# giuvecchio/PyPBR

Hardware: AMD Instinct MI355X
Metric: Mpixels/s Cook-Torrance eval, 4K maps (higher is better)
Workload: dtype f32

## Files before the change

### __graft_entry__.py

```python
import os
import subprocess
import sys

ROOT = os.path.dirname(os.path.abspath(__file__))
if ROOT not in sys.path:
    sys.path.insert(0, ROOT)


def build() -> None:
    subprocess.check_call(["make", "-s", "-j4", "-C", os.path.join(ROOT, "pypbr_amd", "csrc")])
    subprocess.check_call(["make", "-s", "-C", os.path.join(ROOT, "pypbr_amd", "csrc"), "torch_ops"])
    subprocess.check_call(["make", "-s", "-C", os.path.join(ROOT, "oracle")])
    boxcal_src, boxcal_so = os.path.join(ROOT, "tools", "boxcal.hip"), os.path.join(ROOT, "tools", "libboxcal.so")
    if not os.path.exists(boxcal_so) or os.path.getmtime(boxcal_so) < os.path.getmtime(boxcal_src):
        try:
            subprocess.check_call([os.environ.get("HIPCC", "/opt/rocm/bin/hipcc"), "-O3", "--offload-arch=gfx950", "-shared", "-fPIC", boxcal_src, "-o", boxcal_so])
        except (OSError, subprocess.CalledProcessError) as e:
            print("warning: tools/libboxcal.so (bench-side calibration helper, optional) did not build: %s" % e, file=sys.stderr)
    sys.path.insert(0, os.path.join(ROOT, "tools"))
    import check_isa
    report = check_isa.check()
    print("ISA check ok: %d hand-scheduled kernel instantiations; %s" % (sum(1 for r in report if "<" in r.split("vgpr")[0]), report[-1][:120]))
    import pypbr_amd
    from pypbr_amd import _native
    lib = _native.lib()
    for sym in _native.EXPORTS:
        getattr(lib, sym)
    assert lib.pbr_abi_version() == _native.ABI_VERSION
    from pypbr_amd import torch_ops
    assert torch_ops.available(), "pypbr_amd/_pbr_torch_ops.so did not build or load"
    import torch
    for op in ("cook_torrance", "cook_torrance_backward", "fold_gradient", "srgb_to_linear", "linear_to_srgb",
               "metallic_to_diffuse_specular", "diffuse_specular_to_basecolor_metallic", "colour_backward",
               "metallic_to_diffuse_specular_backward", "diffuse_specular_to_basecolor_metallic_backward", "resize", "resize_backward",
               "normal_from_height", "normal_from_height_backward", "normal_transform", "normal_transform_backward",
               "remap_planes", "remap_planes_backward"):
        getattr(torch.ops.pbr_hip, op)
    print("build ok: %s (ABI %d), pypbr_amd %s" % (_native.LIB_PATH, lib.pbr_abi_version(), pypbr_amd.__version__))


def smoke() -> None:
    import torch
    sys.path.insert(0, os.path.join(ROOT, "oracle"))
    import torch_oracle
    from pypbr_amd.materials import BasecolorMetallicMaterial
    from pypbr_amd.models import CookTorranceBRDF

    assert torch.cuda.is_available(), "smoke() needs a ROCm device"
    g = torch.Generator().manual_seed(2024)
    H, W = 96, 128
    albedo = torch.rand(3, H, W, generator=g)
    nxy = torch.rand(2, H, W, generator=g) - 0.5
    normal = torch.cat([nxy, torch.ones(1, H, W)], 0)
    normal = normal / normal.norm(dim=0, keepdim=True)
    rough = torch.rand(1, H, W, generator=g) * 0.85 + 0.15
    metal = torch.rand(1, H, W, generator=g)
    view, light, inten = torch.tensor([0.0, 0.0, 1.0]), torch.tensor([0.1, 0.1, 1.0]), torch.tensor([1.0, 1.0, 1.0])

    mat = BasecolorMetallicMaterial(albedo=albedo, normal=normal, roughness=rough, metallic=metal).to("cuda:0")
    out = CookTorranceBRDF(light_type="point")(mat, view, light, inten, 1.0)
    torch.cuda.synchronize()
    assert out.shape == (3, H, W) and out.device.type == "cuda"
    ref = torch_oracle.cook_torrance(albedo, normal, rough, metal, None, view=view, light=light, intensity=inten,
                                     light_type="point", light_size=1.0)
    err = (out.cpu() - ref).abs().max().item()
    print("smoke: max |hip - oracle| = %.3e over %d values" % (err, ref.numel()))
    assert err <= 1e-5, err


if __name__ == "__main__":
    build()
    if len(sys.argv) > 1 and sys.argv[1] == "smoke":
        smoke()
```

### pypbr_amd/_caches.py

```python
import os
import threading
import weakref
from typing import Optional

import torch

CACHING = {"device_maps": False, "parameters": False, "decode_verdicts": False}
for _tok, _key in (("maps", "device_maps"), ("params", "parameters"), ("decode", "decode_verdicts")):
    if _tok in os.environ.get("PBR_CACHE", "").split(","):
        CACHING[_key] = True


def set_caching(device_maps: Optional[bool] = None, parameters: Optional[bool] = None, decode_verdicts: Optional[bool] = None) -> dict:
    old = dict(CACHING)
    for key, v in (("device_maps", device_maps), ("parameters", parameters), ("decode_verdicts", decode_verdicts)):
        if v is not None:
            CACHING[key] = bool(v)
    return old


def version_of(t: torch.Tensor):
    try:
        return None if t.is_inference() else t._version
    except RuntimeError:
        return None


def weak_refs(tensors):
    return tuple(None if t is None else weakref.ref(t) for t in tensors)


def same_tensors(refs, tensors) -> bool:
    return len(refs) == len(tensors) and all((r is None and t is None) or (r is not None and r() is t) for r, t in zip(refs, tensors))


def host_values(v):
    if isinstance(v, torch.Tensor):
        return None if v.is_cuda or v.requires_grad else v.tolist()
    if isinstance(v, (list, tuple)):
        return [list(r) if isinstance(r, (list, tuple)) else r for r in v]
    return None


class VersionMemo:

    def __init__(self, limit: int = 64):
        self.limit, self._entries = limit, {}

    def get(self, t, version):
        e = self._entries.get(id(t))
        return e[2] if e is not None and e[0]() is t and e[1] == version else None

    def put(self, t, version, payload):
        for k in [k for k, e in self._entries.items() if e[0]() is None]:
            del self._entries[k]
        if len(self._entries) >= self.limit:
            self._entries.clear()
        self._entries[id(t)] = (weakref.ref(t), version, payload)

    def __len__(self):
        return len(self._entries)

    def clear(self):
        self._entries.clear()


class ValueMemo:

    def __init__(self, limit: int = 256):
        self.limit, self._entries = limit, {}

    def get(self, key, make):
        hit = self._entries.get(key)
        if hit is None:
            hit = make()
            if len(self._entries) >= self.limit:
                self._entries.clear()
            self._entries[key] = hit
        return hit

    def __len__(self):
        return len(self._entries)

    def clear(self):
        self._entries.clear()


class KeptPlan:
    __slots__ = ("plan", "maps", "values", "lock", "out_shape")

    def __init__(self, plan, maps, values, out_shape=None):
        self.plan, self.maps, self.values, self.out_shape = plan, weak_refs(maps), values, out_shape
        self.lock = threading.Lock()

    @classmethod
    def adopt(cls, plan, maps, values, out_shape=None):
        if plan._param_block is not None or not all(p is None or (t is not None and p.data_ptr() == t.data_ptr()) for p, t in zip(plan._keep, maps)):
            return None
        plan._keep = ()
        return cls(plan, maps, values, out_shape)

    def describes(self, maps) -> bool:
        return same_tensors(self.maps, maps)

    def try_acquire(self) -> bool:
        return self.lock.acquire(False)

    def release(self):
        self.lock.release()

    def refresh(self, values) -> bool:
        if values != self.values:
            if not self.plan.refill(*values):
                return False
            self.values = values
        return True
```

### pypbr_amd/models.py

```python
import collections
import os
import weakref
from abc import ABC
from typing import Optional

import torch
import torch.nn as nn
from torch import Tensor

from . import _native
from . import functional as F_
from ._caches import KeptPlan, host_values, same_tensors, weak_refs
from .materials import MaterialBase, _normalised


DEVICE_CACHE_CAP = int(os.environ.get("PBR_DEVICE_CACHE_CAP", str(4 << 30)))
_DEVICE_CACHES = collections.OrderedDict()


def _touch_device_cache(material):
    if id(material) in _DEVICE_CACHES:
        _DEVICE_CACHES.move_to_end(id(material))


def _register_device_cache(material, nbytes):
    _DEVICE_CACHES.pop(id(material), None)
    for key in [k for k, (ref, _) in _DEVICE_CACHES.items() if ref() is None or "_device_cache" not in ref().__dict__]:
        del _DEVICE_CACHES[key]
    _DEVICE_CACHES[id(material)] = (weakref.ref(material), nbytes)
    total = sum(n for _, n in _DEVICE_CACHES.values())
    while total > DEVICE_CACHE_CAP and len(_DEVICE_CACHES) > 1:
        _, (ref, n) = _DEVICE_CACHES.popitem(last=False)
        if ref() is not None:
            ref().__dict__.pop("_device_cache", None)
        total -= n


def _upload_together(tensors, compute):
    host = [i for i, t in enumerate(tensors) if t is not None and t.device.type == "cpu"]
    moved = [None if t is None else (t if t.device == compute or t.device.type == "cpu" else t.to(compute)) for t in tensors]
    if host:
        views, _ = F_.upload_packed([tensors[i] for i in host], compute)
        for i, v in zip(host, views):
            moved[i] = v
    return tuple(moved)


class BRDFModel(nn.Module, ABC):
    """Abstract base class for BRDF models (cooktorrance.py:27-30)."""


class CookTorranceBRDF(BRDFModel):

    def __init__(self, light_type: str = "point", override_device: torch.device = None):
        super().__init__()
        self.light_type = light_type.lower()
        if self.light_type not in ["directional", "point"]:
            raise ValueError(
                f"Unsupported light_type: {self.light_type}. Must be 'directional' or 'point'."
            )
        self.override_device = override_device

    @staticmethod
    def _staged(material, maps, blend, compute):
        tensors = tuple(maps) + tuple(blend or ())
        if any(t is not None and t.requires_grad for t in tensors):
            moved = tuple(None if t is None else t.to(compute) for t in tensors)
            return moved[:5], (None if blend is None else moved[5:])
        versions = tuple(None if t is None else F_.version_of(t) for t in tensors)
        wanted = (F_.CACHING["device_maps"] or material.__dict__.get("_cache_on_device", False))
        cacheable = wanted and all(v is not None for t, v in zip(tensors, versions) if t is not None)
        at, seen, refs, moved = (material.__dict__.get("_device_cache") if cacheable else None) or (None, None, (), None)
        if moved is not None and at == compute and seen == versions and same_tensors(refs, tensors):
            _touch_device_cache(material)
        else:
            moved = _upload_together(tensors, compute)
            if cacheable:
                material.__dict__["_device_cache"] = (compute, versions, weak_refs(tensors), moved)
                _register_device_cache(material, sum(t.numel() * t.element_size() for t in moved if t is not None))
        return moved[:5], (None if blend is None else moved[5:])

    PLAN_REUSE = True

    def _reuse_plan(self, material, view_dir, light, intensity, light_size, return_srgb):
        d = material.__dict__
        store = d.get("_store")
        if store is None or d.get("_lazy_blend") is not None or d.get("_raw_normal") or self.override_device is not None:
            return None
        vals = (host_values(view_dir), host_values(light), host_values(intensity))
        if vals[0] is None or vals[1] is None or vals[2] is None:
            return None
        albedo, normal, rough = store.get("albedo"), store.get("normal", False), store.get("roughness")
        metallic = store.get("metallic")
        specular = store.get("specular") if metallic is None else None
        if (albedo is None or normal is False or rough is None or (metallic is None and specular is None) or not albedo.is_cuda
                or albedo.device != material.device):
            return None
        maps = (albedo, normal, rough, metallic, specular)
        grad = torch.is_grad_enabled()
        for t in maps:
            if t is not None and (t.device != albedo.device or t.dtype.itemsize > 4 or not t.is_floating_point() or (grad and t.requires_grad)
                                  or t.stride(-1) != 1 or t.stride(-2) != t.shape[-1]):
                return None
        key = (self.light_type, light_size, bool(return_srgb), bool(material.albedo_is_srgb), bool(getattr(material, "specular_is_srgb", True)),
               d.get("_lazy_tile", (1, 1)),
               tuple((id(t), t.data_ptr(), t.shape, t.dtype, t.stride()) if t is not None else None for t in maps))
        kept_key, kept = d.get("_plan_cache") or (None, None)
        if kept is not None and (kept_key != key or not kept.describes(maps)):
            d.pop("_plan_cache", None)
            kept = None
        if kept is None:
            if d.get("_plan_seen") != key:
                d["_plan_seen"] = key
                return None
            return key
        if not kept.try_acquire():
            return None
        plan = kept.plan
        try:
            if not kept.refresh(vals):
                return key
            dev = plan.device
            out = torch.empty(kept.out_shape, dtype=torch.float32, device=dev)
            plan.out = out
            plan.desc.out = out.data_ptr()
            if torch.cuda.current_device() == dev.index:
                plan.launch()
            else:
                with torch.cuda.device(dev):
                    plan.launch()
            return out[0] if plan._squeeze else out
        finally:
            plan.out = None
            kept.release()

    def forward(self, material, view_dir: Tensor, light_dir_or_position: Tensor, light_intensity: Tensor,
                light_size: Optional[float] = None, return_srgb: bool = True) -> Tensor:
        reuse_key = None
        if self.PLAN_REUSE and isinstance(material, MaterialBase):
            got = self._reuse_plan(material, view_dir, light_dir_or_position, light_intensity, light_size, return_srgb)
            if isinstance(got, torch.Tensor):
                return got
            reuse_key = got
        out_device = _normalised(self.override_device or material.device)

        pending = material.__dict__.get("_lazy_blend")
        blend = None
        if pending is not None:
            first, (second, mask) = material.__dict__["_store"], pending
            albedo, normal, roughness = first["albedo"], first["normal"], first["roughness"]
            metallic, specular = first.get("metallic"), None
            if metallic is None:
                specular = first["specular"]
            specular_is_srgb = bool(getattr(material, "specular_is_srgb", True))
            blend = (second["albedo"], second["normal"], second["roughness"], second.get("metallic") if metallic is not None else None,
                     second.get("specular") if metallic is None else None, mask)
        else:
            store = material.__dict__.get("_store") if isinstance(material, MaterialBase) else None
            if store is not None and material._has_pending():
                store = {**store, **material._resident(keep=False)}

            def probe(name):
                if store is None:
                    return getattr(material, name)
                if name not in store:
                    raise AttributeError(f"'{type(material).__name__}' object has no attribute '{name}'")
                return store[name]

            def has(name):
                return (name in store) if store is not None else hasattr(material, name)

            roughness = probe("roughness")
            normal = probe("normal")
            metallic = specular = None
            specular_is_srgb = True
            if has("metallic") and probe("metallic") is not None:
                metallic = probe("metallic")
            elif has("specular") and probe("specular") is not None:
                specular = probe("specular")
                specular_is_srgb = bool(getattr(material, "specular_is_srgb", True))
            else:
                raise ValueError("Material must have either 'metallic' or 'specular' property.")
            albedo = store.get("albedo") if store is not None else material._maps.get("albedo")
            if albedo is None:
                raise AttributeError(f"'{type(material).__name__}' material has no albedo map")

        if out_device.type == "cuda":
            compute = out_device
        else:
            _native.require_device()
            compute = torch.device("cuda", torch.cuda.current_device())

        maps = (albedo, normal, roughness, metallic, specular)
        if any(t is not None and t.device != compute for t in maps + (blend or ())):
            maps, blend = self._staged(material, maps, blend, compute)
        kw = dict(view_dir=view_dir, light=light_dir_or_position, light_intensity=light_intensity, light_type=self.light_type,
                  light_size=light_size, albedo_is_srgb=bool(material.albedo_is_srgb), specular_is_srgb=specular_is_srgb,
                  return_srgb=return_srgb, tile=getattr(material, "lazy_tile", (1, 1)))
        if reuse_key is not None and blend is None and albedo.numel() > 0:
            plan = F_.plan_cook_torrance(*maps, **kw)
            with torch.cuda.device(plan.device):
                color = plan.launch()
            kept = KeptPlan.adopt(plan, maps, (host_values(view_dir), host_values(light_dir_or_position), host_values(light_intensity)),
                                  tuple(plan.out.shape))
            if kept is not None:
                material.__dict__["_plan_cache"] = (reuse_key, kept)
            plan.out = None
            return color
        color = F_.cook_torrance(*maps, blend=blend, **kw)
        if color.device == out_device:
            return color
        return F_.to_host(color, out_device) if out_device.type == "cpu" else color.to(out_device)
```

### pypbr_amd/torch_ops.py

```python
import os

import torch

_HERE = os.path.dirname(os.path.abspath(__file__))
LIB_PATH = os.path.join(_HERE, "_pbr_torch_ops.so")
_loaded = None


def available() -> bool:
    global _loaded
    if _loaded is None:
        _loaded = False
        if os.environ.get("PBR_NO_TORCH_OPS") != "1" and os.path.exists(LIB_PATH):
            from . import _native
            _native.lib()
            try:
                torch.ops.load_library(LIB_PATH)
                _register()
                _loaded = True
            except (OSError, RuntimeError) as e:
                import warnings
                warnings.warn("pypbr_amd: %s does not load against torch %s (%s); using the ctypes binding of libpbr_hip.so. "
                              "Rebuild with `make -C pypbr_amd/csrc torch_ops`." % (LIB_PATH, torch.__version__, str(e).splitlines()[0]),
                              RuntimeWarning, stacklevel=2)
    return _loaded


def _out_extent(albedo, tile_y, tile_x, y_offset, rows):
    B, _, H, W = albedo.shape
    if tile_y == 1 and tile_x == 1:
        return B, H, W
    return B, (rows if rows > 0 else tile_y * H - y_offset), tile_x * W


def _register():
    lib = torch.library

    @lib.register_fake("pbr_hip::cook_torrance")
    def _(albedo, normal, roughness, metallic, specular, view_dir, lights, intensities, light_size, light_type, albedo_is_srgb,
          specular_is_srgb, convert_to_diffuse_specular, return_srgb, y_offset=0, height_total=0, tile_y=1, tile_x=1, rows=0,
          half_result=False):
        B, H, W = _out_extent(albedo, tile_y, tile_x, y_offset, rows)
        return albedo.new_empty((B, 3, H, W), dtype=torch.float16 if half_result else torch.float32)

    @lib.register_fake("pbr_hip::cook_torrance_backward")
    def _(grad_out, albedo, normal, roughness, metallic, specular, view_dir, lights, intensities, light_size, light_type,
          albedo_is_srgb, specular_is_srgb, convert_to_diffuse_specular, return_srgb, y_offset, height_total, tile_y, tile_x, rows,
          want_albedo, want_normal, want_roughness, want_metallic, want_specular, want_params):
        B, H, W = _out_extent(albedo, tile_y, tile_x, y_offset, rows)
        maps = [t for t in (albedo, normal, roughness, metallic, specular) if t is not None]
        shared = B > 1 and any(t.shape[0] == 1 for t in maps)
        if (tile_y, tile_x) != (1, 1) and not want_params and not shared:
            H, W = albedo.shape[-2:]

        def buf(want, c):
            return albedo.new_empty((B, c, H, W)) if want else albedo.new_empty((0,))
        n_lights = lights.numel() // 3
        return (buf(want_albedo, 3), buf(want_normal and normal is not None, 3), buf(want_roughness, 1),
                buf(want_metallic and metallic is not None, 1), buf(want_specular and metallic is None, 3),
                albedo.new_empty((3 + 6 * n_lights,) if want_params else (0,), dtype=torch.float32))

    @lib.register_fake("pbr_hip::fold_gradient")
    def _(src, h, w, fold_batch):
        return src.new_empty((1 if fold_batch else src.shape[0], src.shape[1], h, w))

    for name in ("srgb_to_linear", "linear_to_srgb"):
        lib.register_fake("pbr_hip::" + name)(lambda texture: torch.empty_like(texture))
    lib.register_fake("pbr_hip::metallic_to_diffuse_specular")(
        lambda albedo, metallic, albedo_is_srgb: (torch.empty_like(albedo), torch.empty_like(albedo)))
    lib.register_fake("pbr_hip::diffuse_specular_to_basecolor_metallic")(
        lambda diffuse, specular, albedo_is_srgb: (torch.empty_like(diffuse), torch.empty_like(diffuse)))

    lib.register_fake("pbr_hip::colour_backward")(lambda texture, grad_out, to_linear: torch.empty_like(texture))
    lib.register_fake("pbr_hip::metallic_to_diffuse_specular_backward")(
        lambda albedo, metallic, g_diffuse, g_specular, albedo_is_srgb: (torch.empty_like(albedo), torch.empty_like(metallic)))
    lib.register_fake("pbr_hip::diffuse_specular_to_basecolor_metallic_backward")(
        lambda diffuse, specular, g_basecolor, g_metallic, albedo_is_srgb: (torch.empty_like(diffuse), torch.empty_like(specular)))
    lib.register_fake("pbr_hip::resize")(lambda texture, h_out, w_out, antialias: texture.new_empty(tuple(texture.shape[:-2]) + (h_out, w_out)))
    lib.register_fake("pbr_hip::resize_backward")(
        lambda grad_out, h_in, w_in, antialias: grad_out.new_empty(tuple(grad_out.shape[:-2]) + (h_in, w_in), dtype=torch.float32))

    def colour_autograd(name, to_linear):
        def setup(ctx, inputs, output):
            ctx.save_for_backward(inputs[0])

        def backward(ctx, grad_out):
            (x,) = ctx.saved_tensors
            return torch.ops.pbr_hip.colour_backward(x, grad_out, to_linear)
        lib.register_autograd("pbr_hip::" + name, backward, setup_context=setup)
    colour_autograd("srgb_to_linear", True)
    colour_autograd("linear_to_srgb", False)

    def pair_autograd(name):
        def setup(ctx, inputs, output):
            ctx.save_for_backward(inputs[0], inputs[1])
            ctx.flag = inputs[2]

        def backward(ctx, g0, g1):
            x, y = ctx.saved_tensors
            gx, gy = getattr(torch.ops.pbr_hip, name + "_backward")(x, y, g0, g1, ctx.flag)
            return (gx if ctx.needs_input_grad[0] else None, gy.to(y.dtype) if ctx.needs_input_grad[1] else None, None)
        lib.register_autograd("pbr_hip::" + name, backward, setup_context=setup)
    pair_autograd("metallic_to_diffuse_specular")
    pair_autograd("diffuse_specular_to_basecolor_metallic")

    def resize_setup(ctx, inputs, output):
        ctx.geom = (inputs[0].shape[-2], inputs[0].shape[-1], inputs[3])

    def resize_backward(ctx, grad_out):
        h, w, antialias = ctx.geom
        return torch.ops.pbr_hip.resize_backward(grad_out, h, w, antialias), None, None, None
    lib.register_autograd("pbr_hip::resize", resize_backward, setup_context=resize_setup)

    def _normals_of(height):
        return height.new_empty((3,) + tuple(height.shape[-2:]) if height.dim() < 4 else (height.shape[0], 3) + tuple(height.shape[-2:]))
    lib.register_fake("pbr_hip::normal_from_height")(lambda height, scale, directx: _normals_of(height))
    lib.register_fake("pbr_hip::normal_from_height_backward")(
        lambda height, grad_normal, scale, directx: height.new_empty(height.shape, dtype=torch.float32))
    lib.register_fake("pbr_hip::normal_transform")(lambda normal, m00, m01, m10, m11, renormalize: torch.empty_like(normal))
    lib.register_fake("pbr_hip::normal_transform_backward")(
        lambda normal, grad_out, m00, m01, m10, m11, renormalize: torch.empty_like(normal, dtype=torch.float32))

    def nfh_setup(ctx, inputs, output):
        ctx.save_for_backward(inputs[0])
        ctx.args = tuple(inputs[1:])

    def nfh_backward(ctx, grad_out):
        (height,) = ctx.saved_tensors
        return torch.ops.pbr_hip.normal_from_height_backward(height, grad_out, *ctx.args).to(height.dtype), None, None
    lib.register_autograd("pbr_hip::normal_from_height", nfh_backward, setup_context=nfh_setup)

    def transform_setup(ctx, inputs, output):
        ctx.save_for_backward(inputs[0])
        ctx.args = tuple(inputs[1:])

    def transform_backward(ctx, grad_out):
        (normal,) = ctx.saved_tensors
        return (torch.ops.pbr_hip.normal_transform_backward(normal, grad_out, *ctx.args).to(normal.dtype),) + (None,) * 5
    lib.register_autograd("pbr_hip::normal_transform", transform_backward, setup_context=transform_setup)

    lib.register_fake("pbr_hip::remap_planes")(
        lambda texture, y_offset, y_step, x_offset, x_step, negate_mask, h_out, w_out: texture.new_empty(tuple(texture.shape[:-2]) + (h_out, w_out)))
    lib.register_fake("pbr_hip::remap_planes_backward")(
        lambda grad_out, h_src, w_src, y_offset, y_step, x_offset, x_step, negate_mask:
        grad_out.new_empty(tuple(grad_out.shape[:-2]) + (h_src, w_src), dtype=torch.float32))

    def remap_setup(ctx, inputs, output):
        ctx.geom = (inputs[0].shape[-2], inputs[0].shape[-1]) + tuple(inputs[1:6])
        ctx.dtype = inputs[0].dtype

    def remap_backward(ctx, grad_out):
        return (torch.ops.pbr_hip.remap_planes_backward(grad_out, *ctx.geom).to(ctx.dtype),) + (None,) * 7
    lib.register_autograd("pbr_hip::remap_planes", remap_backward, setup_context=remap_setup)

    names = ("albedo", "normal", "roughness", "metallic", "specular", "view_dir", "lights", "intensities")

    def setup_context(ctx, inputs, output):
        tensors, rest = inputs[:8], tuple(inputs[8:])
        assert len(rest) == 12, "pbr_hip::cook_torrance takes 8 tensors and 12 scalars"
        ctx.rest = rest
        ctx.present = [t is not None for t in tensors]
        ctx.save_for_backward(*[t for t in tensors if t is not None])
        if output.dtype != torch.float32:
            ctx.half = True

    def backward(ctx, grad_out):
        if getattr(ctx, "half", False):
            raise NotImplementedError("gradients need a float32 result (fp16 maps are fine: their gradients come back in fp16)")
        saved = list(ctx.saved_tensors)
        tensors = [saved.pop(0) if p else None for p in ctx.present]
        albedo, normal, roughness, metallic, specular, view_dir, lights, intensities = tensors
        (light_size, light_type, a_srgb, s_srgb, convert, r_srgb, y_offset, height_total, tile_y, tile_x, rows, _half) = ctx.rest
        need = ctx.needs_input_grad
        want_params = bool(need[5] or need[6] or need[7])
        ga, gn, gr, gm, gs, gp = torch.ops.pbr_hip.cook_torrance_backward(
            grad_out, albedo, normal, roughness, metallic, specular, view_dir, lights, intensities, light_size, light_type, a_srgb,
            s_srgb, convert, r_srgb, y_offset, height_total, tile_y, tile_x, rows, bool(need[0]), bool(need[1] and normal is not None),
            bool(need[2]), bool(need[3] and metallic is not None), bool(need[4] and specular is not None and metallic is None),
            want_params)
        B, _, H, W = albedo.shape
        tiled = (tile_y, tile_x) != (1, 1)
        grads = []
        for g, t, needed in zip((ga, gn, gr, gm, gs), tensors[:5], need[:5]):
            if not needed or t is None or g.numel() == 0:
                grads.append(None)
                continue
            shared = B > 1 and t.shape[0] == 1
            if tiled and tuple(g.shape[-2:]) == (H, W) and not shared:
                grads.append(g)
                continue
            if tiled and grad_out.shape[-2] != tile_y * H:
                raise NotImplementedError("gradients of a tiled evaluation with light / view gradients or batch-shared maps need the whole output, not a row band")
            if tiled or shared:
                g = torch.ops.pbr_hip.fold_gradient(g, H, W, shared)
            grads.append(g)
        L = lights.numel() // 3
        pg = [None, None, None]
        if want_params:
            def like(g, t, lights_many):
                if g.dim() == 2 and t.numel() == 3 and lights_many:
                    g = g.sum(dim=0)
                return g.reshape(t.shape).to(device=t.device, dtype=t.dtype)
            if need[5]:
                pg[0] = like(gp[0:3], view_dir, False)
            if need[6]:
                pg[1] = like(gp[3:3 + 3 * L].reshape(L, 3), lights, False)
            if need[7]:
                pg[2] = like(gp[3 + 3 * L:].reshape(L, 3), intensities, L > 1)
        return (*grads, *pg, *([None] * 12))

    lib.register_autograd("pbr_hip::cook_torrance", backward, setup_context=setup_context)
```

Before: 145,600.

## Add native C++ hit path for repeated Cook-Torrance calls on kept plans

Adds a pybind11 KeptCall object that, on a repeated render call with the same material tensors, validates tensor identity and host light/view parameters in C++. It then writes them into the kept descriptor and launches the kernel directly, bypassing the Python plan-reuse path. The aim is to cut per-call Python dispatch overhead on the cached-plan path. It adds locking interplay between the Python and native locks, plus more build and ABI surface.

```diff
diff --git a/__graft_entry__.py b/__graft_entry__.py
--- a/__graft_entry__.py
+++ b/__graft_entry__.py
@@ -9,7 +9,7 @@
 
 def build() -> None:
     subprocess.check_call(["make", "-s", "-j4", "-C", os.path.join(ROOT, "pypbr_amd", "csrc")])
-    subprocess.check_call(["make", "-s", "-C", os.path.join(ROOT, "pypbr_amd", "csrc"), "torch_ops"])
+    subprocess.check_call(["make", "-s", "-j2", "-C", os.path.join(ROOT, "pypbr_amd", "csrc"), "torch_ops"])
     subprocess.check_call(["make", "-s", "-C", os.path.join(ROOT, "oracle")])
     boxcal_src, boxcal_so = os.path.join(ROOT, "tools", "boxcal.hip"), os.path.join(ROOT, "tools", "libboxcal.so")
     if not os.path.exists(boxcal_so) or os.path.getmtime(boxcal_so) < os.path.getmtime(boxcal_src):
@@ -29,6 +29,7 @@
     assert lib.pbr_abi_version() == _native.ABI_VERSION
     from pypbr_amd import torch_ops
     assert torch_ops.available(), "pypbr_amd/_pbr_torch_ops.so did not build or load"
+    assert torch_ops.kept_call_register() is not None
     import torch
     for op in ("cook_torrance", "cook_torrance_backward", "fold_gradient", "srgb_to_linear", "linear_to_srgb",
                "metallic_to_diffuse_specular", "diffuse_specular_to_basecolor_metallic", "colour_backward",
diff --git a/pypbr_amd/_caches.py b/pypbr_amd/_caches.py
--- a/pypbr_amd/_caches.py
+++ b/pypbr_amd/_caches.py
@@ -87,26 +87,41 @@
 
 
 class KeptPlan:
-    __slots__ = ("plan", "maps", "values", "lock", "out_shape")
+    __slots__ = ("plan", "maps", "values", "lock", "out_shape", "native", "scalars")
 
     def __init__(self, plan, maps, values, out_shape=None):
         self.plan, self.maps, self.values, self.out_shape = plan, weak_refs(maps), values, out_shape
         self.lock = threading.Lock()
+        self.native = self.scalars = None
 
     @classmethod
-    def adopt(cls, plan, maps, values, out_shape=None):
+    def adopt(cls, plan, maps, values, out_shape=None, register=None, scalars=None):
         if plan._param_block is not None or not all(p is None or (t is not None and p.data_ptr() == t.data_ptr()) for p, t in zip(plan._keep, maps)):
             return None
         plan._keep = ()
-        return cls(plan, maps, values, out_shape)
+        kept = cls(plan, maps, values, out_shape)
+        if register is not None:
+            kept.native, kept.scalars = register(plan, maps, out_shape), scalars
+        return kept
 
     def describes(self, maps) -> bool:
         return same_tensors(self.maps, maps)
 
     def try_acquire(self) -> bool:
-        return self.lock.acquire(False)
+        if not self.lock.acquire(False):
+            return False
+        if self.native is not None:
+            got = self.native.try_lock()
+            if not got:
+                self.lock.release()
+                return False
+            if got == 2:
+                self.values = None
+        return True
 
     def release(self):
+        if self.native is not None:
+            self.native.unlock()
         self.lock.release()
 
     def refresh(self, values) -> bool:
diff --git a/pypbr_amd/csrc/kept_call.cpp b/pypbr_amd/csrc/kept_call.cpp
--- /dev/null
+++ b/pypbr_amd/csrc/kept_call.cpp
@@ -0,0 +1,199 @@
+#include <ATen/ATen.h>
+#include <c10/core/DeviceGuard.h>
+#include <c10/core/GradMode.h>
+#include <c10/hip/HIPStream.h>
+#include <pybind11/pybind11.h>
+#include <pybind11/stl.h>
+#include <torch/csrc/autograd/python_variable.h>
+
+#include <array>
+#include <atomic>
+#include <cstdint>
+#include <optional>
+#include <vector>
+
+#include "../../include/pbr_hip.h"
+
+namespace py = pybind11;
+
+namespace {
+
+using at::Tensor;
+
+py::object &status_raiser() {
+    static py::object *fn = new py::object();
+    return *fn;
+}
+
+struct MapIdentity {
+    std::optional<c10::weak_intrusive_ptr<c10::TensorImpl>> impl;
+    const void *data = nullptr;
+    int64_t dim = 0;
+    std::array<int64_t, 4> sizes{}, strides{};
+    c10::ScalarType dtype = c10::ScalarType::Undefined;
+
+    bool matches(PyObject *o, const c10::Device &device, bool grad_mode) const {
+        if (o == Py_None) return !impl.has_value();
+        if (!impl.has_value() || !THPVariable_Check(o)) return false;
+        const Tensor &t = THPVariable_Unpack(o);
+        if (t.unsafeGetTensorImpl() != impl->_unsafe_get_target()) return false;
+        if (t.dim() != dim || t.scalar_type() != dtype || t.device() != device || (grad_mode && t.requires_grad())) return false;
+        const auto sz = t.sizes(), st = t.strides();
+        for (int64_t i = 0; i < dim; ++i)
+            if (sz[i] != sizes[i] || st[i] != strides[i]) return false;
+        return t.data_ptr() == data;
+    }
+};
+
+int host_rows(PyObject *o, bool many, float (*dst)[3]) {
+    if (!THPVariable_Check(o)) return 0;
+    const Tensor &t = THPVariable_Unpack(o);
+    if (!t.device().is_cpu() || t.layout() != at::kStrided || t.requires_grad() || !t.is_contiguous()) return 0;
+    int64_t rows;
+    if (t.dim() == 1 && t.size(0) == 3) rows = 1;
+    else if (many && t.dim() == 2 && t.size(1) == 3 && t.size(0) >= 1 && t.size(0) <= PBR_MAX_LIGHTS) rows = t.size(0);
+    else return 0;
+    if (t.scalar_type() == at::kFloat) {
+        const float *p = t.const_data_ptr<float>();
+        for (int64_t i = 0; i < rows; ++i)
+            for (int c = 0; c < 3; ++c) dst[i][c] = p[3 * i + c];
+    } else if (t.scalar_type() == at::kDouble) {
+        const double *p = t.const_data_ptr<double>();
+        for (int64_t i = 0; i < rows; ++i)
+            for (int c = 0; c < 3; ++c) dst[i][c] = (float)p[3 * i + c];
+    } else {
+        return 0;
+    }
+    return (int)rows;
+}
+
+class KeptCall {
+  public:
+    KeptCall(py::object owner, pbr_render_desc *desc, std::array<MapIdentity, 5> maps, c10::Device device, std::vector<int64_t> out_shape,
+             bool squeeze)
+        : owner_(std::move(owner)), desc_(desc), maps_(std::move(maps)), device_(device), out_shape_(std::move(out_shape)), squeeze_(squeeze) {}
+
+    struct Parameters {
+        float view[1][3], lights[PBR_MAX_LIGHTS][3], intensities[PBR_MAX_LIGHTS][3];
+        int intensity_rows;
+    };
+
+    bool decide(PyObject *const given[5], PyObject *view_dir, PyObject *light, PyObject *intensity, Parameters &p) const {
+        const bool grad_mode = at::GradMode::is_enabled();
+        for (int i = 0; i < 5; ++i)
+            if (!maps_[i].matches(given[i], device_, grad_mode)) return false;
+        const int L = desc_->n_lights;
+        if (host_rows(view_dir, false, p.view) != 1 || host_rows(light, true, p.lights) != L) return false;
+        p.intensity_rows = host_rows(intensity, true, p.intensities);
+        return p.intensity_rows == L || p.intensity_rows == 1;
+    }
+
+    bool follows(py::handle albedo, py::handle normal, py::handle roughness, py::handle metallic, py::handle specular, py::handle view_dir,
+                 py::handle light, py::handle intensity) const {
+        PyObject *given[5] = {albedo.ptr(), normal.ptr(), roughness.ptr(), metallic.ptr(), specular.ptr()};
+        Parameters p;
+        return decide(given, view_dir.ptr(), light.ptr(), intensity.ptr(), p);
+    }
+
+    py::object call(py::handle albedo, py::handle normal, py::handle roughness, py::handle metallic, py::handle specular, py::handle view_dir,
+                    py::handle light, py::handle intensity) {
+        PyObject *given[5] = {albedo.ptr(), normal.ptr(), roughness.ptr(), metallic.ptr(), specular.ptr()};
+        Parameters p;
+        if (!device_.is_cuda() || !decide(given, view_dir.ptr(), light.ptr(), intensity.ptr(), p)) return py::none();
+        if (busy_.exchange(true, std::memory_order_acquire)) return py::none();
+        struct Release {
+            std::atomic<bool> &flag;
+            ~Release() { flag.store(false, std::memory_order_release); }
+        } release{busy_};
+        const int L = desc_->n_lights;
+        for (int c = 0; c < 3; ++c) desc_->view_dir[c] = p.view[0][c];
+        for (int i = 0; i < L; ++i)
+            for (int c = 0; c < 3; ++c) {
+                desc_->lights[i][c] = p.lights[i][c];
+                desc_->intensities[i][c] = p.intensities[p.intensity_rows == 1 ? 0 : i][c];
+            }
+        written_ = true;
+        const c10::DeviceGuard guard(device_);
+        Tensor out = at::empty(out_shape_, at::TensorOptions().dtype(at::kFloat).device(device_));
+        desc_->out = out.data_ptr();
+        const int rc = pbr_cook_torrance(desc_, c10::hip::getCurrentHIPStream(device_.index()).stream());
+        if (rc != PBR_OK) {
+            status_raiser()(rc);
+            throw std::runtime_error(pbr_error_string(rc));
+        }
+        ++hits_;
+        return py::reinterpret_steal<py::object>(THPVariable_Wrap(squeeze_ ? out.select(0, 0) : out));
+    }
+
+    int64_t hits() const { return hits_; }
+
+    int try_lock() {
+        if (busy_.exchange(true, std::memory_order_acquire)) return 0;
+        const bool w = written_;
+        written_ = false;
+        return w ? 2 : 1;
+    }
+    void unlock() { busy_.store(false, std::memory_order_release); }
+
+  private:
+    py::object owner_;
+    pbr_render_desc *desc_;
+    std::array<MapIdentity, 5> maps_;
+    c10::Device device_;
+    std::vector<int64_t> out_shape_;
+    bool squeeze_;
+    bool written_ = false;
+    int64_t hits_ = 0;
+    std::atomic<bool> busy_{false};
+};
+
+py::object register_kept_call(py::object owner, uintptr_t address, py::tuple maps, std::vector<int64_t> out_shape, bool squeeze) {
+    auto *desc = reinterpret_cast<pbr_render_desc *>(address);
+    if (desc == nullptr || maps.size() != 5 || desc->abi_version != PBR_HIP_ABI_VERSION || desc->out_dtype != PBR_F32 ||
+        desc->device_params != nullptr || desc->n_lights < 1 || desc->n_lights > PBR_MAX_LIGHTS || desc->out_batch_stride != 0 ||
+        desc->out_channel_stride != 0)
+        return py::none();
+    int64_t numel = 1;
+    for (int64_t s : out_shape) numel *= s;
+    if (out_shape.size() != 4 || numel <= 0 || out_shape[1] != 3 || (squeeze && out_shape[0] != 1)) return py::none();
+    const pbr_map *slots[5] = {&desc->albedo, &desc->normal, &desc->roughness, &desc->metallic, &desc->specular};
+    std::array<MapIdentity, 5> ids;
+    std::optional<c10::Device> device;
+    for (int i = 0; i < 5; ++i) {
+        py::handle o = maps[i];
+        if (o.is_none()) {
+            if (i == 0 || i == 2 || slots[i]->data != nullptr) return py::none();
+            continue;
+        }
+        if (!THPVariable_Check(o.ptr())) return py::none();
+        const Tensor &t = THPVariable_Unpack(o.ptr());
+        const int64_t n = t.dim();
+        if (t.layout() != at::kStrided || (t.scalar_type() != at::kFloat && t.scalar_type() != at::kHalf) || n < 3 || n > 4 ||
+            t.stride(n - 1) != 1 || t.stride(n - 2) != t.size(n - 1) || t.data_ptr() != slots[i]->data)
+            return py::none();
+        if (!device.has_value()) device = t.device();
+        if (t.device() != *device) return py::none();
+        MapIdentity &m = ids[i];
+        m.impl.emplace(t.getIntrusivePtr());
+        m.data = t.data_ptr();
+        m.dim = n;
+        for (int64_t k = 0; k < n; ++k) { m.sizes[k] = t.size(k); m.strides[k] = t.stride(k); }
+        m.dtype = t.scalar_type();
+    }
+    return py::cast(new KeptCall(std::move(owner), desc, std::move(ids), *device, std::move(out_shape), squeeze),
+                    py::return_value_policy::take_ownership);
+}
+
+}
+
+PYBIND11_MODULE(_pbr_torch_ops, m) {
+    m.doc() = "native hit path of CookTorranceBRDF.__call__ on a kept plan (pypbr_amd/csrc/kept_call.cpp)";
+    py::class_<KeptCall>(m, "KeptCall")
+        .def("call", &KeptCall::call)
+        .def("follows", &KeptCall::follows)
+        .def_property_readonly("hits", &KeptCall::hits)
+        .def("try_lock", &KeptCall::try_lock)
+        .def("unlock", &KeptCall::unlock);
+    m.def("register_kept_call", &register_kept_call);
+    m.def("set_status_raiser", [](py::object fn) { status_raiser() = std::move(fn); });
+}
diff --git a/pypbr_amd/models.py b/pypbr_amd/models.py
--- a/pypbr_amd/models.py
+++ b/pypbr_amd/models.py
@@ -10,6 +10,7 @@
 
 from . import _native
 from . import functional as F_
+from . import torch_ops
 from ._caches import KeptPlan, host_values, same_tensors, weak_refs
 from .materials import MaterialBase, _normalised
 
@@ -81,12 +82,24 @@
         return moved[:5], (None if blend is None else moved[5:])
 
     PLAN_REUSE = True
+    NATIVE_CALL = True
 
     def _reuse_plan(self, material, view_dir, light, intensity, light_size, return_srgb):
         d = material.__dict__
         store = d.get("_store")
         if store is None or d.get("_lazy_blend") is not None or d.get("_raw_normal") or self.override_device is not None:
             return None
+        if self.NATIVE_CALL:
+            cached = d.get("_plan_cache")
+            if cached is not None and cached[1].native is not None:
+                kept = cached[1]
+                if kept.scalars == (self.light_type, light_size, bool(return_srgb), bool(material.albedo_is_srgb),
+                                    bool(getattr(material, "specular_is_srgb", True)), d.get("_lazy_tile", (1, 1)), material.device):
+                    metallic = store.get("metallic")
+                    out = kept.native.call(store.get("albedo"), store.get("normal", False), store.get("roughness"), metallic,
+                                           store.get("specular") if metallic is None else None, view_dir, light, intensity)
+                    if out is not None:
+                        return out
         vals = (host_values(view_dir), host_values(light), host_values(intensity))
         if vals[0] is None or vals[1] is None or vals[2] is None:
             return None
@@ -202,7 +215,7 @@
             with torch.cuda.device(plan.device):
                 color = plan.launch()
             kept = KeptPlan.adopt(plan, maps, (host_values(view_dir), host_values(light_dir_or_position), host_values(light_intensity)),
-                                  tuple(plan.out.shape))
+                                  tuple(plan.out.shape), register=torch_ops.kept_call_register(), scalars=reuse_key[:6] + (material.device,))
             if kept is not None:
                 material.__dict__["_plan_cache"] = (reuse_key, kept)
             plan.out = None
diff --git a/pypbr_amd/torch_ops.py b/pypbr_amd/torch_ops.py
--- a/pypbr_amd/torch_ops.py
+++ b/pypbr_amd/torch_ops.py
@@ -5,10 +5,11 @@
 _HERE = os.path.dirname(os.path.abspath(__file__))
 LIB_PATH = os.path.join(_HERE, "_pbr_torch_ops.so")
 _loaded = None
+_module = None
 
 
 def available() -> bool:
-    global _loaded
+    global _loaded, _module
     if _loaded is None:
         _loaded = False
         if os.environ.get("PBR_NO_TORCH_OPS") != "1" and os.path.exists(LIB_PATH):
@@ -17,13 +18,36 @@
             try:
                 torch.ops.load_library(LIB_PATH)
                 _register()
+                _module = _import_module()
                 _loaded = True
-            except (OSError, RuntimeError) as e:
+            except (OSError, RuntimeError, ImportError) as e:
                 import warnings
                 warnings.warn("pypbr_amd: %s does not load against torch %s (%s); using the ctypes binding of libpbr_hip.so. "
                               "Rebuild with `make -C pypbr_amd/csrc torch_ops`." % (LIB_PATH, torch.__version__, str(e).splitlines()[0]),
                               RuntimeWarning, stacklevel=2)
     return _loaded
+
+
+def _import_module():
+    import importlib.util
+    from . import _native
+    spec = importlib.util.spec_from_file_location(__package__ + "._pbr_torch_ops", LIB_PATH)
+    module = importlib.util.module_from_spec(spec)
+    spec.loader.exec_module(module)
+    module.set_status_raiser(_native.check)
+    return module
+
+
+def kept_call_register():
+    if not available():
+        return None
+    import ctypes
+
+    def register(plan, maps, out_shape):
+        if out_shape is None or getattr(plan, "_blend", None) is not None or plan.desc.tuning:
+            return None
+        return _module.register_kept_call(plan.desc, ctypes.addressof(plan.desc), tuple(maps), list(out_shape), bool(plan._squeeze))
+    return register
 
 
 def _out_extent(albedo, tile_y, tile_x, y_offset, rows):
```

After: 145,700 (median of 3 runs). No clear change (+0.1%).
